# duowuyms/MANSY_ImmersiveVideoStreaming

Measured on AMD Instinct MI355X. Metric: viewport-trajectories/sec (VP train), higher is better.
Workload: dtype f32; 1 GPU; VP Transformer train step (fwd+loss+bwd+AdamW), B=4096/GPU synthetic torus-walk trajectories len 21 (hist 10 + cur 1 + pred 10), d=512, 8 heads, 2+2 layers, dropout on, fp32 MFMA, decoder recurrence as two half-batches on two streams; two_stream=True, global_batch=4096, parallelism=dp1

## Files before the change

mansy_immersivevideostreaming_amd/csrc/vp_engine.hip:

```cpp
#include <stdlib.h>
#include <algorithm>
#include <string>
#include <vector>
#include "mansy_kernels.h"
#include "../../include/mansy_hip.h"

namespace {

constexpr int MAXL = 8;

inline uint32_t site_pe_src() { return 1u; }
inline uint32_t site_enc(int l, int k) { return 100u + l * 8 + k; }
inline uint32_t site_pe_tgt(int i) { return 1000u + i; }
inline uint32_t site_dec(int l, int i, int k) { return 10000u + (l * 64 + i) * 8 + k; }

struct LinearP { const float* w = nullptr; const float* b = nullptr; float* gw = nullptr; float* gb = nullptr; };
typedef LinearP NormP;
struct EncLayerP { LinearP in_proj, out_proj, lin1, lin2; NormP n1, n2; };
struct DecLayerP { LinearP sa_in, sa_out, ca_in, ca_out, lin1, lin2; NormP n1, n2, n3; };
struct VPParams {
  LinearP emb; EncLayerP enc[MAXL]; NormP enc_norm; DecLayerP dec[MAXL]; NormP dec_norm;
  LinearP conv; NormP bn; LinearP pred;
};

struct ParamInfo { std::string name; long long numel; int ndim; long long shape[4]; };

void add_param(std::vector<ParamInfo>& v, const std::string& name, long long a, long long b = 0, long long c = 0) {
  ParamInfo p; p.name = name; p.shape[0] = a; p.shape[1] = b; p.shape[2] = c; p.shape[3] = 0;
  p.ndim = c ? 3 : (b ? 2 : 1);
  p.numel = a * (b ? b : 1) * (c ? c : 1);
  v.push_back(p);
}

std::vector<ParamInfo> param_table(const mansy_vp_config& c) {
  std::vector<ParamInfo> v;
  const long long d = c.d_model, f = c.d_ff;
  const bool hb = c.has_bias != 0;
  add_param(v, "embedding.linear.weight", d, c.in_ch);
  add_param(v, "embedding.linear.bias", d);
  auto mha = [&](const std::string& p) {
    add_param(v, p + "in_proj_weight", 3 * d, d);
    if (hb) add_param(v, p + "in_proj_bias", 3 * d);
    add_param(v, p + "out_proj.weight", d, d);
    if (hb) add_param(v, p + "out_proj.bias", d);
  };
  auto lin = [&](const std::string& p, long long o, long long i) {
    add_param(v, p + ".weight", o, i);
    if (hb) add_param(v, p + ".bias", o);
  };
  auto norm = [&](const std::string& p) {
    add_param(v, p + ".weight", d);
    if (hb) add_param(v, p + ".bias", d);
  };
  for (int l = 0; l < c.n_enc; ++l) {
    const std::string p = "transformer.encoder.layers." + std::to_string(l) + ".";
    mha(p + "self_attn.");
    lin(p + "linear1", f, d); lin(p + "linear2", d, f);
    norm(p + "norm1"); norm(p + "norm2");
  }
  norm("transformer.encoder.norm");
  for (int l = 0; l < c.n_dec; ++l) {
    const std::string p = "transformer.decoder.layers." + std::to_string(l) + ".";
    mha(p + "self_attn."); mha(p + "multihead_attn.");
    lin(p + "linear1", f, d); lin(p + "linear2", d, f);
    norm(p + "norm1"); norm(p + "norm2"); norm(p + "norm3");
  }
  norm("transformer.decoder.norm");
  add_param(v, "transformer.distill_layer.downConv.weight", d, d, 3);
  add_param(v, "transformer.distill_layer.downConv.bias", d);
  add_param(v, "transformer.distill_layer.norm.weight", d);
  add_param(v, "transformer.distill_layer.norm.bias", d);
  add_param(v, "predictor.0.weight", c.in_ch, d);
  add_param(v, "predictor.0.bias", c.in_ch);
  return v;
}

void bind_params(const mansy_vp_config& c, const float* const* params, float* const* grads, VPParams& P) {
  int k = 0;
  const bool hb = c.has_bias != 0;
  auto nextw = [&](LinearP& L, bool bias) {
    L.w = params[k]; L.gw = grads ? grads[k] : nullptr; ++k;
    if (bias) { L.b = params[k]; L.gb = grads ? grads[k] : nullptr; ++k; }
  };
  nextw(P.emb, true);
  for (int l = 0; l < c.n_enc; ++l) {
    EncLayerP& e = P.enc[l];
    nextw(e.in_proj, hb); nextw(e.out_proj, hb); nextw(e.lin1, hb); nextw(e.lin2, hb); nextw(e.n1, hb); nextw(e.n2, hb);
  }
  nextw(P.enc_norm, hb);
  for (int l = 0; l < c.n_dec; ++l) {
    DecLayerP& e = P.dec[l];
    nextw(e.sa_in, hb); nextw(e.sa_out, hb); nextw(e.ca_in, hb); nextw(e.ca_out, hb);
    nextw(e.lin1, hb); nextw(e.lin2, hb); nextw(e.n1, hb); nextw(e.n2, hb); nextw(e.n3, hb);
  }
  nextw(P.dec_norm, hb);
  nextw(P.conv, true);
  nextw(P.bn, true);
  nextw(P.pred, true);
}

struct EncBuf { float *qkv, *P, *ao, *z1, *m1, *r1, *y1, *h, *z2, *m2, *r2, *y2; };
struct DecBuf {
  float *memkv, *qkv, *P1, *ao1, *z1, *m1, *r1, *y1, *qc, *P2, *ao2, *z2, *m2, *r2, *y2, *h, *z3, *m3, *r3, *y3;
  float *dqkv, *dbr1, *dqc, *dbr2, *da, *dbr3, *dmemkv;
  float *dao2, *dS2, *Pk2;
  float *dao1, *dS1, *Pk1;
};
struct Work {
  float *src6, *cur6, *fut6, *pred_bt, *dpred_bt;
  float *x0; EncBuf enc[MAXL]; float *enc_out, *me, *re;
  float *col, *conv, *bn_mean, *bn_rstd, *mem; unsigned char* argmax; double* stats; double* dis_part;
  float *tok_all, *emb_all; DecBuf dec[MAXL]; float *dec_out, *md, *rd;
  float *t_enc, *t_dec;
  float *g_a, *g_b, *g_c, *g_wide, *g_ff;
  float *s_a, *s_b, *s_c, *s_tok;
  float *dE_all, *dz_all, *dmem;
  float *lnp_dec, *lnp_enc;
  double* loss_acc;
  unsigned short *wpl, *wpl_t;
  long long wpl_stride;
  const float* fbase; unsigned short* img;
};
struct BufInfo { std::string name; size_t off; size_t bytes; };

struct Layout {
  std::vector<BufInfo> bufs;
  size_t total = 0;
  char* base = nullptr;
  void* add(const std::string& name, size_t bytes) {
    const size_t off = (total + 255) & ~size_t(255);
    total = off + bytes;
    bufs.push_back({name, off, bytes});
    return base ? (void*)(base + off) : nullptr;
  }
  float* f(const std::string& name, size_t n) { return (float*)add(name, n * sizeof(float)); }
};

void build_layout(const mansy_vp_config& c, Layout& L, Work& W) {
  const size_t B = c.B, S = c.S, T = c.T, d = c.d_model, f = c.d_ff, H = c.n_head, C6 = c.in_ch;
  const size_t M = (S - 1) / 2 + 1, N = B * S, TB = T * B;
  W.src6 = L.f("src6", N * C6); W.cur6 = L.f("cur6", B * C6); W.fut6 = L.f("fut6", TB * C6);
  W.pred_bt = L.f("pred_bt", TB * C6); W.dpred_bt = L.f("dpred_bt", TB * C6);
  W.x0 = L.f("enc.x0", N * d);
  for (int l = 0; l < c.n_enc; ++l) {
    const std::string p = "enc" + std::to_string(l) + ".";
    EncBuf& e = W.enc[l];
    e.qkv = L.f(p + "qkv", N * 3 * d); e.P = L.f(p + "P", B * H * S * S); e.ao = L.f(p + "ao", N * d);
    e.z1 = L.f(p + "z1", N * d); e.m1 = L.f(p + "m1", N); e.r1 = L.f(p + "r1", N); e.y1 = L.f(p + "y1", N * d);
    e.h = L.f(p + "h", N * f);
    e.z2 = L.f(p + "z2", N * d); e.m2 = L.f(p + "m2", N); e.r2 = L.f(p + "r2", N); e.y2 = L.f(p + "y2", N * d);
  }
  W.enc_out = L.f("enc.out", N * d); W.me = L.f("enc.me", N); W.re = L.f("enc.re", N);
  W.col = L.f("dis.col", N * 3 * d); W.conv = L.f("dis.conv", N * d);
  W.bn_mean = L.f("dis.bn_mean", d); W.bn_rstd = L.f("dis.bn_rstd", d);
  W.mem = L.f("mem", B * M * d);
  W.argmax = (unsigned char*)L.add("dis.argmax", B * M * d);
  W.stats = (double*)L.add("dis.stats", 6 * d * sizeof(double));
  W.dis_part = (double*)L.add("dis.part", (size_t)MANSY_DISTILL_PARTS * 2 * d * sizeof(double));
  W.tok_all = L.f("tok_all", (T + 1) * B * C6);
  W.emb_all = L.f("dec.emb", TB * d);
  for (int l = 0; l < c.n_dec; ++l) {
    const std::string p = "dec" + std::to_string(l) + ".";
    DecBuf& e = W.dec[l];
    e.memkv = L.f(p + "memkv", B * M * 2 * d);
    e.qkv = L.f(p + "qkv", TB * 3 * d); e.P1 = L.f(p + "P1", TB * H * T); e.ao1 = L.f(p + "ao1", TB * d);
    e.z1 = L.f(p + "z1", TB * d); e.m1 = L.f(p + "m1", TB); e.r1 = L.f(p + "r1", TB); e.y1 = L.f(p + "y1", TB * d);
    e.qc = L.f(p + "qc", TB * d); e.P2 = L.f(p + "P2", TB * H * M); e.ao2 = L.f(p + "ao2", TB * d);
    e.z2 = L.f(p + "z2", TB * d); e.m2 = L.f(p + "m2", TB); e.r2 = L.f(p + "r2", TB); e.y2 = L.f(p + "y2", TB * d);
    e.h = L.f(p + "h", TB * f);
    e.z3 = L.f(p + "z3", TB * d); e.m3 = L.f(p + "m3", TB); e.r3 = L.f(p + "r3", TB); e.y3 = L.f(p + "y3", TB * d);
    e.dqkv = L.f(p + "dqkv", TB * 3 * d); e.dbr1 = L.f(p + "dbr1", TB * d); e.dqc = L.f(p + "dqc", TB * d);
    e.dbr2 = L.f(p + "dbr2", TB * d); e.da = L.f(p + "da", TB * f); e.dbr3 = L.f(p + "dbr3", TB * d);
    e.dmemkv = L.f(p + "dmemkv", B * M * 2 * d);
    e.dao2 = L.f(p + "dao2", TB * d); e.dS2 = L.f(p + "dS2", TB * H * M); e.Pk2 = L.f(p + "Pk2", TB * H * M);
    e.dao1 = L.f(p + "dao1", TB * d); e.dS1 = L.f(p + "dS1", TB * H * T); e.Pk1 = L.f(p + "Pk1", TB * H * T);
  }
  W.dec_out = L.f("dec.out", TB * d); W.md = L.f("dec.md", TB); W.rd = L.f("dec.rd", TB);
  W.t_enc = L.f("tmp.t_enc", N * d); W.t_dec = L.f("tmp.t_dec", B * d);
  W.g_a = L.f("tmp.g_a", N * d); W.g_b = L.f("tmp.g_b", N * d); W.g_c = L.f("tmp.g_c", N * d);
  W.g_wide = L.f("tmp.g_wide", N * 3 * d); W.g_ff = L.f("tmp.g_ff", N * f);
  W.s_a = L.f("tmp.s_a", B * d); W.s_b = L.f("tmp.s_b", B * d); W.s_c = L.f("tmp.s_c", B * d);
  W.s_tok = L.f("tmp.s_tok", B * C6);
  W.dE_all = L.f("dec.dE", TB * d); W.dz_all = L.f("dec.dz", TB * C6); W.dmem = L.f("dmem", B * M * d);
  W.lnp_dec = L.f("lnp.dec", (size_t)2 * (3 * c.n_dec + 1) * mansy_ln_bwd_parts((int)B) * 2 * d);
  W.lnp_enc = L.f("lnp.enc", (size_t)(2 * c.n_enc + 1) * mansy_ln_bwd_parts((int)N) * 2 * d);
  W.loss_acc = (double*)L.add("loss_acc", 64);
  size_t wtot = 0;
  for (const ParamInfo& pi : param_table(c))
    if (pi.ndim >= 2 && pi.shape[0] * (pi.numel / pi.shape[0]) == pi.numel && pi.numel / pi.shape[0] >= 32 && pi.shape[0] >= 32)
      wtot += ((size_t)pi.numel + 63) / 64 * 64;
  W.wpl_stride = (long long)wtot;
  W.wpl = (unsigned short*)L.add("wplanes", wtot * 2 * sizeof(unsigned short));
  W.wpl_t = (unsigned short*)L.add("wplanes_t", wtot * 2 * sizeof(unsigned short));
  const size_t floats_above = (L.total + 3) / 4;
  W.fbase = (const float*)L.base;
  W.img = (unsigned short*)L.add("bf16_images", floats_above * sizeof(unsigned short));
}

int check_cfg(const mansy_vp_config* c) {
  MANSY_REQUIRE(c, "vp: null config");
  MANSY_REQUIRE(c->B >= 1 && c->S >= 1 && c->S <= 16 && c->T >= 1 && c->T <= 16, "vp: need B>=1, 1<=S,T<=16 (got B=%d S=%d T=%d)", c->B, c->S, c->T);
  MANSY_REQUIRE(c->n_head >= 1 && c->d_model % c->n_head == 0 && c->d_model / c->n_head <= 64, "vp: d_model/n_head must be an integer <= 64");
  MANSY_REQUIRE(c->d_model % 4 == 0 && c->d_ff % 4 == 0, "vp: d_model and d_ff must be multiples of 4");
  MANSY_REQUIRE(c->n_enc >= 1 && c->n_enc <= MAXL && c->n_dec >= 1 && c->n_dec <= MAXL, "vp: 1..%d layers supported", MAXL);
  MANSY_REQUIRE(c->in_ch >= 1 && c->in_ch <= 8 && c->in_ch % 3 == 0, "vp: in_ch must be 3*in_channel <= 8");
  MANSY_REQUIRE(c->max_len >= c->S && c->max_len >= c->T, "vp: positional table too short");
  MANSY_REQUIRE(c->p_pe >= 0.f && c->p_pe < 1.f && c->p_drop >= 0.f && c->p_drop < 1.f, "vp: dropout p outside [0,1)");
  MANSY_REQUIRE(c->precision == 0 || c->precision == 1 || c->precision == 3 || c->precision == 6, "vp: precision must be MANSY_PREC_F32 (0), _BF16 (1), _BF16X3 (3) or _BF16X6 (6), got %d", c->precision);
  return MANSY_OK;
}

#define RC(expr) do { int _rc = (expr); if (_rc) return _rc; } while (0)

struct Eng {
  const mansy_vp_config& c;
  VPParams P;
  Work W;
  hipStream_t st;
  bool train;
  uint32_t seed;
  int B, S, T, d, f, H, dh, M, N, TB, C6;
  float drop_scale;

  Eng(const mansy_vp_config& cfg, hipStream_t s, bool tr, uint32_t sd) : c(cfg), st(s), train(tr), seed(sd) {
    wtab.n = 0;
    prec = c.precision;
    B = c.B; S = c.S; T = c.T; d = c.d_model; f = c.d_ff; H = c.n_head; dh = d / H; M = (S - 1) / 2 + 1;
    N = B * S; TB = T * B; C6 = c.in_ch;
    drop_scale = (train && c.p_drop > 0.f) ? 1.f / (1.f - c.p_drop) : 1.f;
  }
  MansyWPlaneTab wtab; int prec = 0;
  bool s16 = false;
  unsigned short* im(const float* p) const { return s16 ? W.img + (p - W.fbase) : nullptr; }
// ... 108 lines not shown
  }
  AttnShape self_shape(int i, int nb = -1) const {
    AttnShape s; s.nb = nb < 0 ? B : nb; s.H = H; s.Lq = 1; s.Lk = i + 1; s.dh = dh;
    s.q_bs = 3 * d; s.q_rs = 0; s.k_bs = s.v_bs = 3 * d; s.k_rs = s.v_rs = (long long)B * 3 * d;
    s.o_bs = d; s.o_rs = 0; s.scale = 1.f / sqrtf((float)dh);
    return s;
  }
  AttnShape cross_shape(int nb = -1) const {
    AttnShape s; s.nb = nb < 0 ? B : nb; s.H = H; s.Lq = 1; s.Lk = M; s.dh = dh;
    s.q_bs = d; s.q_rs = 0; s.k_bs = s.v_bs = (long long)M * 2 * d; s.k_rs = s.v_rs = 2 * d;
    s.o_bs = d; s.o_rs = 0; s.scale = 1.f / sqrtf((float)dh);
    return s;
  }

  int forward(const float* src, const float* cur, const float* pe, float* bn_rm, float* bn_rv, long long* bn_nbt, float* pred_bt) {
    RC(prepare_planes());
    RC(mansy_launch_embed_fwd(src, C6, P.emb.w, P.emb.b, pe, W.x0, N, d, S, -1, dr(site_pe_src(), c.p_pe), st, im(W.x0)));
    const float* x = W.x0;
    for (int l = 0; l < c.n_enc; ++l) {
      const EncLayerP& p = P.enc[l]; EncBuf& e = W.enc[l];
      RC(lin_fwd(x, N, d, p.in_proj.w, p.in_proj.b, 3 * d, e.qkv, 0, mansy_no_drop()));
      RC(mansy_launch_attn_fwd(e.qkv, e.qkv + d, e.qkv + 2 * d, e.ao, e.P, enc_shape(), dr(site_enc(l, 0), c.p_drop), st, attn_im()));
      RC(lin_fwd(e.ao, N, d, p.out_proj.w, p.out_proj.b, d, e.z1, 0, dr(site_enc(l, 1), c.p_drop), x));
      RC(ln_of(e.z1, p.n1, e.y1, e.m1, e.r1, N));
      RC(lin_fwd(e.y1, N, d, p.lin1.w, p.lin1.b, f, e.h, 1, dr(site_enc(l, 2), c.p_drop), nullptr, 2));
      RC(lin_fwd(e.h, N, f, p.lin2.w, p.lin2.b, d, e.z2, 0, dr(site_enc(l, 3), c.p_drop), e.y1));
      RC(ln_of(e.z2, p.n2, e.y2, e.m2, e.r2, N));
      x = e.y2;
    }
    RC(ln_fwd(x, nullptr, P.enc_norm, nullptr, W.enc_out, W.me, W.re, N));
    RC(mansy_launch_im2col3(W.enc_out, W.col, B, S, d, st, im(W.col)));
    RC(lin_fwd(W.col, N, 3 * d, P.conv.w, P.conv.b, d, W.conv, 0, mansy_no_drop()));
    DistillShape ds = {B, S, M, d, c.bn_sync_world > 1 ? c.bn_sync_world : 1, c.bn_sync_fn, c.bn_sync_user};
    RC(mansy_launch_distill_fwd(W.conv, P.bn.w, P.bn.b, bn_rm, bn_rv, bn_nbt, W.bn_mean, W.bn_rstd, W.mem, W.argmax, W.stats, ds,
                                train ? 1 : 0, c.bn_eps, c.bn_momentum, st, W.dis_part, im(W.mem)));
    for (int l = 0; l < c.n_dec; ++l) {
      const DecLayerP& p = P.dec[l];
      RC(lin_fwd(W.mem, B * M, d, p.ca_in.w + (size_t)d * d, p.ca_in.b ? p.ca_in.b + d : nullptr, 2 * d, W.dec[l].memkv, 0, mansy_no_drop(), nullptr, 1));
    }
    MANSY_HIP_CHECK(hipMemcpyAsync(W.tok_all, cur, sizeof(float) * B * C6, hipMemcpyDeviceToDevice, st));
    const bool fuse_tail = mansy_dec_tail_ok(d, C6) != 0;
    const bool split = split_ok();
    const int h0 = split ? B / 2 : B;
    if (split) RC(fork());
    for (int i = 0; i < T; ++i) {
      RC(dec_fwd_step(i, 0, h0, pe, pred_bt, fuse_tail));
      if (split) { hipStream_t keep = st; st = st2; int rc = dec_fwd_step(i, h0, B - h0, pe, pred_bt, fuse_tail); st = keep; RC(rc); }
    }
    if (split) RC(join());
    return MANSY_OK;
  }

  hipStream_t st2 = nullptr;
  bool split_ok() const { return B % 2 == 0 && ((c.two_stream == 1 && B >= 2048) || (c.two_stream == 2 && B >= 256)); }
  int fork() {
    static thread_local hipStream_t s2 = nullptr; static thread_local hipEvent_t ev_f = nullptr;
    if (!s2) { MANSY_HIP_CHECK(hipStreamCreateWithFlags(&s2, hipStreamNonBlocking)); MANSY_HIP_CHECK(hipEventCreateWithFlags(&ev_f, hipEventDisableTiming)); }
    st2 = s2;
    MANSY_HIP_CHECK(hipEventRecord(ev_f, st));
    MANSY_HIP_CHECK(hipStreamWaitEvent(st2, ev_f, 0));
    return MANSY_OK;
  }
  int join() {
    static thread_local hipEvent_t ev_j = nullptr;
    if (!ev_j) MANSY_HIP_CHECK(hipEventCreateWithFlags(&ev_j, hipEventDisableTiming));
    MANSY_HIP_CHECK(hipEventRecord(ev_j, st2));
    MANSY_HIP_CHECK(hipStreamWaitEvent(st, ev_j, 0));
    return MANSY_OK;
  }

  int dec_fwd_step(int i, int b0, int nb, const float* pe, float* pred_bt, bool fuse_tail) {
    const size_t o = (size_t)i * B + b0;
    const float* tok = W.tok_all + o * C6;
    float* emb = W.emb_all + o * d;
    float* t_dec = W.t_dec + (size_t)b0 * d;
    if (i == 0 || !fuse_tail) RC(mansy_launch_embed_fwd(tok, C6, P.emb.w, P.emb.b, pe, emb, nb, d, 1, i, dr(site_pe_tgt(i), c.p_pe, (size_t)b0 * d), st, im(emb)));
    const float* xi = emb;
    for (int l = 0; l < c.n_dec; ++l) {
      const DecLayerP& p = P.dec[l]; DecBuf& e = W.dec[l];
      float* qkv_i = e.qkv + o * 3 * d;
      const float* kv0 = e.qkv + (size_t)b0 * 3 * d;
      const float* mkv = e.memkv + (size_t)b0 * M * 2 * d;
      RC(lin_fwd(xi, nb, d, p.sa_in.w, p.sa_in.b, 3 * d, qkv_i, 0, mansy_no_drop(), nullptr, 1));
      RC(mansy_launch_attn_fwd(qkv_i, kv0 + d, kv0 + 2 * d, e.ao1 + o * d, e.P1 + o * H * T, self_shape(i, nb),
                               dr(site_dec(l, i, 0), c.p_drop, (size_t)b0 * H * (i + 1)), st, attn_im(true)));
      RC(lin_fwd(e.ao1 + o * d, nb, d, p.sa_out.w, p.sa_out.b, d, e.z1 + o * d, 0, dr(site_dec(l, i, 1), c.p_drop, (size_t)b0 * d), xi));
      RC(ln_of(e.z1 + o * d, p.n1, e.y1 + o * d, e.m1 + o, e.r1 + o, nb));
      RC(lin_fwd(e.y1 + o * d, nb, d, p.ca_in.w, p.ca_in.b, d, e.qc + o * d, 0, mansy_no_drop()));
      RC(mansy_launch_attn_fwd(e.qc + o * d, mkv, mkv + d, e.ao2 + o * d, e.P2 + o * H * M, cross_shape(nb),
                               dr(site_dec(l, i, 2), c.p_drop, (size_t)b0 * H * M), st, attn_im(true)));
      RC(lin_fwd(e.ao2 + o * d, nb, d, p.ca_out.w, p.ca_out.b, d, e.z2 + o * d, 0, dr(site_dec(l, i, 3), c.p_drop, (size_t)b0 * d), e.y1 + o * d));
      RC(ln_of(e.z2 + o * d, p.n2, e.y2 + o * d, e.m2 + o, e.r2 + o, nb));
      RC(lin_fwd(e.y2 + o * d, nb, d, p.lin1.w, p.lin1.b, f, e.h + o * f, 1, dr(site_dec(l, i, 4), c.p_drop, (size_t)b0 * f), nullptr, 2));
      if (fuse_tail && l == c.n_dec - 1) {
        RC(lin_fwd(e.h + o * f, nb, f, p.lin2.w, p.lin2.b, d, t_dec, 0, dr(site_dec(l, i, 5), c.p_drop, (size_t)b0 * d)));
        break;
      }
      RC(lin_fwd(e.h + o * f, nb, f, p.lin2.w, p.lin2.b, d, e.z3 + o * d, 0, dr(site_dec(l, i, 5), c.p_drop, (size_t)b0 * d), e.y2 + o * d));
      RC(ln_of(e.z3 + o * d, p.n3, e.y3 + o * d, e.m3 + o, e.r3 + o, nb));
      xi = e.y3 + o * d;
    }
    if (fuse_tail) {
      const DecLayerP& p = P.dec[c.n_dec - 1]; DecBuf& e = W.dec[c.n_dec - 1];
      MansyDecTailFwd tp;
      tp.a = e.y2 + o * d; tp.b = t_dec; tp.n3_w = p.n3.w; tp.n3_b = p.n3.b; tp.z3 = e.z3 + o * d; tp.y3 = e.y3 + o * d;
      tp.m3 = e.m3 + o; tp.r3 = e.r3 + o;
      tp.dn_w = P.dec_norm.w; tp.dn_b = P.dec_norm.b; tp.dec_out = W.dec_out + o * d; tp.md = W.md + o; tp.rd = W.rd + o;
      tp.pw = P.pred.w; tp.pb = P.pred.b; tp.tok_next = W.tok_all + ((size_t)(i + 1) * B + b0) * C6;
      tp.pred_bt = pred_bt ? pred_bt + ((size_t)b0 * T + i) * C6 : nullptr; tp.pred_stride = (long long)T * C6;
      const bool more = i + 1 < T;
      tp.ew = P.emb.w; tp.eb = P.emb.b; tp.pe_row = pe + (size_t)(i + 1) * d; tp.emb_next = more ? W.emb_all + ((size_t)(i + 1) * B + b0) * d : nullptr;
      tp.edrop = dr(site_pe_tgt(i + 1), c.p_pe, (size_t)b0 * d);
      tp.rows = nb; tp.C = d; tp.C6 = C6; tp.eps = c.ln_eps;
// ... 76 lines not shown
                                          dr(site_dec(l, i, 0), c.p_drop, (size_t)b0 * H * (i + 1)), st, attn_im(true)));
      } else {
        RC(lin_dx(e.dbr1 + o * d, nb, d, p.sa_out.w, d, gt, nullptr, nullptr, 1.f));
        RC(mansy_launch_attn_bwd(qkv_at(e, o), kv0 + d, kv0 + 2 * d, e.P1 + o * H * T, gt, dqkv_i, dkv0 + d, dkv0 + 2 * d,
                                 self_shape(i, nb), dr(site_dec(l, i, 0), c.p_drop, (size_t)b0 * H * (i + 1)), 1, st));
      }
      RC(lin_dx(dqkv_i, nb, 3 * d, p.sa_in.w, d, gx, gz, nullptr, 1.f));
    }
    if (!fuse_head) return mansy_launch_embed_bwd(gx, P.emb.w, W.dE_all + o * d, s_tok, C6, nb, d, dr(site_pe_tgt(i), c.p_pe, bd), st);
    if (i == 0) return mansy_launch_embed_bwd(gx, P.emb.w, W.dE_all + o * d, nullptr, C6, nb, d, dr(site_pe_tgt(0), c.p_pe, bd), st);
    return MANSY_OK;
  }
  const float* qkv_at(const DecBuf& e, size_t o) const { return e.qkv + o * 3 * d; }

  int backward(const float* src, const float* dpred_bt) {
    if (wtab.n == 0) RC(prepare_planes());
    const float ms = drop_scale;
    const bool defer_cross = mansy_attn_deferred_kv_ok(cross_shape(), T) != 0;
    const bool pull_self = mansy_attn_deferred_kv_ok(self_shape(T - 1), T) != 0;
    for (int l = 0; l < c.n_dec; ++l) {
      if (!pull_self) MANSY_HIP_CHECK(hipMemsetAsync(W.dec[l].dqkv, 0, sizeof(float) * (size_t)TB * 3 * d, st));
      if (!defer_cross) MANSY_HIP_CHECK(hipMemsetAsync(W.dec[l].dmemkv, 0, sizeof(float) * (size_t)B * M * 2 * d, st));
    }
    const bool ln_parts = mansy_ln_bwd_partial_ok(d);
    const size_t lnp_set = (size_t)mansy_ln_bwd_parts(B) * 2 * d;
    const int n_ln = 3 * c.n_dec + 1;
    const bool split = split_ok();
    const int h0 = split ? B / 2 : B;
    if (ln_parts) MANSY_HIP_CHECK(hipMemsetAsync(W.lnp_dec, 0, sizeof(float) * (size_t)(split ? 2 : 1) * n_ln * lnp_set, st));
    const bool fuse_head = ln_parts && mansy_dec_tail_ok(d, C6) != 0;
    if (split) RC(fork());
    for (int i = T - 1; i >= 0; --i) {
      RC(dec_bwd_step(i, 0, h0, 0, dpred_bt, defer_cross, pull_self, ln_parts, fuse_head));
      if (split) {
        hipStream_t keep = st; st = st2;
        const int rc = dec_bwd_step(i, h0, B - h0, 1, dpred_bt, defer_cross, pull_self, ln_parts, fuse_head);
        st = keep; RC(rc);
      }
    }
    if (split) RC(join());
    if (ln_parts) {
      for (int half = 0; half < (split ? 2 : 1); ++half) {
        const int np = mansy_ln_bwd_parts(half ? B - h0 : h0);
        float* base = W.lnp_dec + (size_t)half * n_ln * lnp_set;
        for (int l = 0; l < c.n_dec; ++l) {
          ln_pending[ln_n_pending++] = MansyLnReduce{base + (size_t)(3 * l + 0) * lnp_set, np, P.dec[l].n1.gw, P.dec[l].n1.gb};
          ln_pending[ln_n_pending++] = MansyLnReduce{base + (size_t)(3 * l + 1) * lnp_set, np, P.dec[l].n2.gw, P.dec[l].n2.gb};
          ln_pending[ln_n_pending++] = MansyLnReduce{base + (size_t)(3 * l + 2) * lnp_set, np, P.dec[l].n3.gw, P.dec[l].n3.gb};
        }
        ln_pending[ln_n_pending++] = MansyLnReduce{base + (size_t)(3 * c.n_dec) * lnp_set, np, P.dec_norm.gw, P.dec_norm.gb};
      }
      RC(flush_ln());
    }
    const bool side_dw = split && c.bn_sync_world <= 1;
    if (side_dw) RC(fork());
    {
      hipStream_t keep = st;
      if (side_dw) st = st2;
      int rc = mansy_launch_outer_reduce(W.dz_all, C6, W.dec_out, TB, d, P.pred.gw, 0, nullptr, P.pred.gb, st);
      if (!rc) rc = mansy_launch_outer_reduce(W.tok_all, C6, W.dE_all, TB, d, P.emb.gw, 1, P.emb.gb, nullptr, st);
      for (int l = 0; l < c.n_dec && !rc; ++l) {
        const DecLayerP& p = P.dec[l]; DecBuf& e = W.dec[l];
        const float* x_all = l == 0 ? W.emb_all : W.dec[l - 1].y3;
        rc = lin_dw(e.dqkv, x_all, TB, 3 * d, d, p.sa_in.gw, p.sa_in.gb);
        if (!rc) rc = lin_dw(e.dbr1, e.ao1, TB, d, d, p.sa_out.gw, p.sa_out.gb);
        if (!rc) rc = lin_dw(e.dqc, e.y1, TB, d, d, p.ca_in.gw, p.ca_in.gb);
        if (!rc) rc = lin_dw(e.dbr2, e.ao2, TB, d, d, p.ca_out.gw, p.ca_out.gb);
        if (!rc) rc = lin_dw(e.da, e.y2, TB, f, d, p.lin1.gw, p.lin1.gb);
        if (!rc) rc = lin_dw(e.dbr3, e.h, TB, d, f, p.lin2.gw, p.lin2.gb);
      }
      st = keep;
      RC(rc);
    }
    for (int l = 0; l < c.n_dec; ++l) {
      const DecLayerP& p = P.dec[l]; DecBuf& e = W.dec[l];
      if (defer_cross)
        RC(mansy_launch_attn_kvgrad(e.qc, (long long)B * d, e.dao2, (long long)B * d, e.dS2, e.Pk2, e.dmemkv, e.dmemkv + d, cross_shape(), T, 0, st, attn_im()));
      RC(lin_dw(e.dmemkv, W.mem, B * M, 2 * d, d, p.ca_in.gw + (size_t)d * d, p.ca_in.gb ? p.ca_in.gb + d : nullptr, defer_cross));
      RC(lin_dx(e.dmemkv, B * M, 2 * d, p.ca_in.w + (size_t)d * d, d, W.dmem, l == 0 ? nullptr : W.dmem, nullptr, 1.f, 0, defer_cross));
    }
    DistillShape ds = {B, S, M, d, c.bn_sync_world > 1 ? c.bn_sync_world : 1, c.bn_sync_fn, c.bn_sync_user};
    RC(mansy_launch_distill_bwd(W.conv, W.dmem, W.argmax, P.bn.w, P.bn.b, W.bn_mean, W.bn_rstd, W.g_a, W.g_b, P.bn.gw, P.bn.gb, W.stats,
                                ds, st, W.dis_part, im(W.g_b)));
    RC(lin_dw(W.g_b, W.col, N, d, 3 * d, P.conv.gw, P.conv.gb));
    RC(lin_dx(W.g_b, N, d, P.conv.w, 3 * d, W.g_wide, nullptr, nullptr, 1.f));
    RC(mansy_launch_col2im3(W.g_wide, W.g_a, B, S, d, st));
    if (c.bn_sync_world > 1) RC(mansy_bn_sync_invoke(2, c.bn_sync_fn, c.bn_sync_user));
    const float* last = W.enc[c.n_enc - 1].y2;
    RC(ln_bwd(W.g_a, last, W.me, W.re, P.enc_norm, W.g_b, nullptr, mansy_no_drop(), N, -1));
    float* gx = W.g_b; float* gz = W.g_a; float* gt = W.g_c;
    for (int l = c.n_enc - 1; l >= 0; --l) {
      const EncLayerP& p = P.enc[l]; EncBuf& e = W.enc[l];
      const float* x_in = l == 0 ? W.x0 : W.enc[l - 1].y2;
      RC(ln_bwd(gx, e.z2, e.m2, e.r2, p.n2, gz, gt, dr(site_enc(l, 3), c.p_drop), N, -(2 + 2 * l)));
      RC(lin_dw(gt, e.h, N, d, f, p.lin2.gw, p.lin2.gb));
      RC(lin_dx(gt, N, d, p.lin2.w, f, W.g_ff, nullptr, e.h, ms, 2));
      RC(lin_dw(W.g_ff, e.y1, N, f, d, p.lin1.gw, p.lin1.gb));
      RC(lin_dx(W.g_ff, N, f, p.lin1.w, d, gt, gz, nullptr, 1.f));
      RC(ln_bwd(gt, e.z1, e.m1, e.r1, p.n1, gz, gx, dr(site_enc(l, 1), c.p_drop), N, -(3 + 2 * l)));
      RC(lin_dw(gx, e.ao, N, d, d, p.out_proj.gw, p.out_proj.gb));
      RC(lin_dx(gx, N, d, p.out_proj.w, d, gt, nullptr, nullptr, 1.f));
      RC(mansy_launch_attn_bwd(e.qkv, e.qkv + d, e.qkv + 2 * d, e.P, gt, W.g_wide, W.g_wide + d, W.g_wide + 2 * d, enc_shape(),
                               dr(site_enc(l, 0), c.p_drop), 0, st, attn_im()));
      RC(lin_dw(W.g_wide, x_in, N, 3 * d, d, p.in_proj.gw, p.in_proj.gb));
      RC(lin_dx(W.g_wide, N, 3 * d, p.in_proj.w, d, gx, gz, nullptr, 1.f));
    }
    RC(mansy_launch_embed_bwd(gx, P.emb.w, gt, nullptr, C6, N, d, dr(site_pe_src(), c.p_pe), st));
    RC(mansy_launch_outer_reduce(src, C6, gt, N, d, P.emb.gw, 1, P.emb.gb, nullptr, st));
    RC(flush_ln());
    if (side_dw) RC(join());
    return MANSY_OK;
  }
};

int setup(const mansy_vp_config* cfg, void* workspace, Layout& L, Work& W) {
  RC(check_cfg(cfg));
  L.base = (char*)workspace;
  build_layout(*cfg, L, W);
  return MANSY_OK;
}

}

extern "C" {

int mansy_vp_num_params(const mansy_vp_config* cfg) {
  if (check_cfg(cfg)) return MANSY_EINVAL;
  return (int)param_table(*cfg).size();
}

int mansy_vp_param_info(const mansy_vp_config* cfg, int idx, char* name, int name_len, long long* numel, int* ndim, long long shape[4]) {
  RC(check_cfg(cfg));
  const std::vector<ParamInfo> t = param_table(*cfg);
  MANSY_REQUIRE(idx >= 0 && idx < (int)t.size(), "vp_param_info: index %d out of range", idx);
  if (name && name_len > 0) { strncpy(name, t[idx].name.c_str(), name_len - 1); name[name_len - 1] = 0; }
  if (numel) *numel = t[idx].numel;
  if (ndim) *ndim = t[idx].ndim;
  if (shape) for (int i = 0; i < 4; ++i) shape[i] = t[idx].shape[i];
  return MANSY_OK;
}

size_t mansy_vp_workspace_bytes(const mansy_vp_config* cfg) {
  Layout L; Work W;
  if (setup(cfg, nullptr, L, W)) return 0;
  return L.total + 256;
}

int mansy_vp_ws_lookup(const mansy_vp_config* cfg, const char* name, long long* offset_bytes, long long* numel) {
  Layout L; Work W;
  RC(setup(cfg, nullptr, L, W));
  for (const BufInfo& b : L.bufs)
    if (b.name == name) { if (offset_bytes) *offset_bytes = (long long)b.off; if (numel) *numel = (long long)(b.bytes / 4); return MANSY_OK; }
  mansy_set_error("vp_ws_lookup: unknown buffer '%s'", name);
  return MANSY_EINVAL;
}

int mansy_vp_forward(const mansy_vp_config* cfg, const float* const* params, const float* pe, float* bn_running_mean,
                     float* bn_running_var, long long* bn_num_batches, const float* src, const float* cur, float* pred,
                     void* workspace, int train, uint32_t seed, void* stream) {
  MANSY_REQUIRE(params && pe && bn_running_mean && bn_running_var && src && cur && pred && workspace, "vp_forward: null pointer");
  Layout L; Work W;
  RC(setup(cfg, workspace, L, W));
  Eng e(*cfg, (hipStream_t)stream, train != 0, seed);
  e.W = W;
// ... 58 lines not shown
```

mansy_immersivevideostreaming_amd/viewport_prediction/models/mtio.py:

```python
import ctypes
import random
import weakref

import numpy as np
import torch
import torch.nn as nn

from ... import _lib
from ..._lib import VPConfig, check, lib, ptr, stream_ptr

_PE_MAX_LEN = 5000
_N_HEAD = 8
_ATTN_DROPOUT = 0.1


_BN_MODELS = weakref.WeakValueDictionary()


def _bn_sync_callback(which, user):
    try:
        m = _BN_MODELS[int(user or 0)]
        cfg = m._bn_cfg
        if which == 2:
            if m._grad_ready is not None:
# ... 12 lines not shown


_BN_SYNC_CFUNC = _lib.BN_SYNC_FN(_bn_sync_callback)


class _Node(nn.Module):
    """Name-space node so parameters get the reference's dotted state_dict keys."""


def _positional_table(max_len, d_model):
    import math
    pe = torch.zeros(max_len, d_model)
    position = torch.arange(0, max_len).unsqueeze(1)
    div_term = torch.exp(torch.arange(0, d_model, 2) * -(math.log(10000.0) / d_model))
    pe[:, 0::2] = torch.sin(position * div_term)
    pe[:, 1::2] = torch.cos(position * div_term)
    return pe.unsqueeze(0)


class ViewportTransformerMTIO(nn.Module):
    def __init__(self, in_channel, fut_window, d_model, dim_feedforward, num_head=3, num_encoder_layers=2,
                 num_decoder_layers=2, batch_first=True, dropout=0.2, device='cuda', repeat_prob=0.5, seed=1,
                 bias=True):
        super().__init__()
        if not batch_first:
            raise ValueError('only batch_first=True is supported (the reference never uses anything else)')
        if num_head != 3:
            raise ValueError('the HIP MTIO kernels are built for num_head=3 (reference default)')
        self.in_channel = in_channel
        self.num_head = num_head
        self.fut_window = fut_window
        self.d_model = d_model
        self.dim_feedforward = dim_feedforward
        self.num_encoder_layers = num_encoder_layers
        self.num_decoder_layers = num_decoder_layers
        self.dropout_p = float(dropout)
        self.attn_dropout_p = _ATTN_DROPOUT
        self.device = device
        self.repeat_prob = repeat_prob
        self.seed = seed
        self.has_bias = bool(bias)
        self.precision = None
        self._ws = {}
        self._flat_p = None
        self._flat_g = None
        self.bn_sync_world = 1
        self._bn_allreduce = None
        self._grad_ready = None
        self.two_stream = None
        self._build_parameters()
        self._flatten()

    def _cfg(self, B, S, inference=False):
        two = 1 if self.two_stream is None else (2 if self.two_stream else 0)
        if self.precision is not None and self.precision not in _lib.PRECISIONS:
            raise _lib.MansyError(f'unknown precision {self.precision!r}: one of f32, bf16, bf16x3, bf16x6')
        cfg = VPConfig(B=B, S=S, T=self.fut_window, d_model=self.d_model, n_head=_N_HEAD, d_ff=self.dim_feedforward,
                       n_enc=self.num_encoder_layers, n_dec=self.num_decoder_layers, in_ch=self.in_channel * self.num_head,
                       has_bias=int(self.has_bias), p_pe=self.dropout_p, p_drop=self.attn_dropout_p, ln_eps=1e-5, bn_eps=1e-5,
                       bn_momentum=0.1, max_len=_PE_MAX_LEN, bn_sync_world=int(self.bn_sync_world), two_stream=int(two),
                       precision=_lib.resolve_precision(self.precision))
        if self.bn_sync_world > 1:
            cfg.bn_sync_fn = _BN_SYNC_CFUNC
            cfg.bn_sync_user = id(self)
        return cfg

    def set_data_parallel(self, world, allreduce=None):
        self.bn_sync_world = int(world)
        if allreduce is None:
            import torch.distributed as dist
            allreduce = dist.all_reduce
        self._bn_allreduce = allreduce
        if self.bn_sync_world > 1:
            _BN_MODELS[id(self)] = self
        else:
            _BN_MODELS.pop(id(self), None)

    def _arm_bn_sync(self, cfg):
        if self.bn_sync_world > 1:
            self._bn_cfg = cfg

    def _param_table(self):
        L = lib()
        cfg = self._cfg(1, 1)
        n = L.mansy_vp_num_params(ctypes.byref(cfg))
        if n <= 0:
            check(-1, 'mansy_vp_num_params')
        out = []
        for i in range(n):
            buf = ctypes.create_string_buffer(160)
            numel, nd, shape = ctypes.c_longlong(), ctypes.c_int(), (ctypes.c_longlong * 4)()
            check(L.mansy_vp_param_info(ctypes.byref(cfg), i, buf, 160, ctypes.byref(numel), ctypes.byref(nd), shape),
                  'mansy_vp_param_info')
            out.append((buf.value.decode(), tuple(shape[:nd.value])))
        return out

    def _set_nested(self, dotted, value, buffer=False):
        parts = dotted.split('.')
        node = self
        for p in parts[:-1]:
            if p not in node._modules:
                node.add_module(p, _Node())
            node = node._modules[p]
        if buffer:
            node.register_buffer(parts[-1], value)
        else:
            node.register_parameter(parts[-1], value)
# ... 337 lines not shown
```

Measured before the change: 185,900 trajectories/s.

## Drive backward post-decoder phase from dependency-tracked two-stream schedule with aside weight grads

New measurement: 186,000 trajectories/s, median of 2. Within noise of the previous version (+0.1%).

```diff
diff --git a/mansy_immersivevideostreaming_amd/csrc/vp_engine.hip b/mansy_immersivevideostreaming_amd/csrc/vp_engine.hip
--- a/mansy_immersivevideostreaming_amd/csrc/vp_engine.hip
+++ b/mansy_immersivevideostreaming_amd/csrc/vp_engine.hip
@@ -3,11 +3,12 @@
 #include <string>
 #include <vector>
 #include "mansy_kernels.h"
+#include "vp_sched.h"
 #include "../../include/mansy_hip.h"
 
 namespace {
 
-constexpr int MAXL = 8;
+constexpr int MAXL = vp_sched::MAXL;
 
 inline uint32_t site_pe_src() { return 1u; }
 inline uint32_t site_enc(int l, int k) { return 100u + l * 8 + k; }
@@ -113,6 +114,7 @@
   float *tok_all, *emb_all; DecBuf dec[MAXL]; float *dec_out, *md, *rd;
   float *t_enc, *t_dec;
   float *g_a, *g_b, *g_c, *g_wide, *g_ff;
+  float *g_x, *g_b2, *g_c2, *g_wide2, *g_ff2;
   float *s_a, *s_b, *s_c, *s_tok;
   float *dE_all, *dz_all, *dmem;
   float *lnp_dec, *lnp_enc;
@@ -179,6 +181,8 @@
   W.t_enc = L.f("tmp.t_enc", N * d); W.t_dec = L.f("tmp.t_dec", B * d);
   W.g_a = L.f("tmp.g_a", N * d); W.g_b = L.f("tmp.g_b", N * d); W.g_c = L.f("tmp.g_c", N * d);
   W.g_wide = L.f("tmp.g_wide", N * 3 * d); W.g_ff = L.f("tmp.g_ff", N * f);
+  W.g_x = L.f("tmp.g_x", N * d); W.g_b2 = L.f("tmp.g_b2", N * d); W.g_c2 = L.f("tmp.g_c2", N * d);
+  W.g_wide2 = L.f("tmp.g_wide2", N * 3 * d); W.g_ff2 = L.f("tmp.g_ff2", N * f);
   W.s_a = L.f("tmp.s_a", B * d); W.s_b = L.f("tmp.s_b", B * d); W.s_c = L.f("tmp.s_c", B * d);
   W.s_tok = L.f("tmp.s_tok", B * C6);
   W.dE_all = L.f("dec.dE", TB * d); W.dz_all = L.f("dec.dz", TB * C6); W.dmem = L.f("dmem", B * M * d);
@@ -393,13 +397,16 @@
   }
 
   hipStream_t st2 = nullptr;
-  bool split_ok() const { return B % 2 == 0 && ((c.two_stream == 1 && B >= 2048) || (c.two_stream == 2 && B >= 256)); }
+  bool split_ok() const { return B % 2 == 0 && ((c.two_stream == 1 && B >= 2048) || ((c.two_stream == 2 || c.two_stream == 3) && B >= 256)); }
+  struct SideRes { hipStream_t s2 = nullptr; hipEvent_t ev_f = nullptr; std::vector<hipEvent_t> pool; };
+  static SideRes& side_res() { static thread_local SideRes r; return r; }
   int fork() {
-    static thread_local hipStream_t s2 = nullptr; static thread_local hipEvent_t ev_f = nullptr;
-    if (!s2) { MANSY_HIP_CHECK(hipStreamCreateWithFlags(&s2, hipStreamNonBlocking)); MANSY_HIP_CHECK(hipEventCreateWithFlags(&ev_f, hipEventDisableTiming)); }
-    st2 = s2;
-    MANSY_HIP_CHECK(hipEventRecord(ev_f, st));
-    MANSY_HIP_CHECK(hipStreamWaitEvent(st2, ev_f, 0));
+    SideRes& r = side_res();
+    if (!r.s2) MANSY_HIP_CHECK(hipStreamCreateWithFlags(&r.s2, hipStreamNonBlocking));
+    if (!r.ev_f) MANSY_HIP_CHECK(hipEventCreateWithFlags(&r.ev_f, hipEventDisableTiming));
+    st2 = r.s2;
+    MANSY_HIP_CHECK(hipEventRecord(r.ev_f, st));
+    MANSY_HIP_CHECK(hipStreamWaitEvent(st2, r.ev_f, 0));
     return MANSY_OK;
   }
   int join() {
@@ -582,64 +589,98 @@
       }
       RC(flush_ln());
     }
-    const bool side_dw = split && c.bn_sync_world <= 1;
-    if (side_dw) RC(fork());
-    {
-      hipStream_t keep = st;
-      if (side_dw) st = st2;
-      int rc = mansy_launch_outer_reduce(W.dz_all, C6, W.dec_out, TB, d, P.pred.gw, 0, nullptr, P.pred.gb, st);
-      if (!rc) rc = mansy_launch_outer_reduce(W.tok_all, C6, W.dE_all, TB, d, P.emb.gw, 1, P.emb.gb, nullptr, st);
-      for (int l = 0; l < c.n_dec && !rc; ++l) {
+    const vp_sched::Sched sch = vp_sched::build(c.n_enc, c.n_dec, split, c.bn_sync_world > 1, defer_cross, c.two_stream == 3);
+    hipEvent_t* ev = nullptr;
+    if (sch.n_events) {
+      SideRes& r = side_res();
+      if (!r.s2) MANSY_HIP_CHECK(hipStreamCreateWithFlags(&r.s2, hipStreamNonBlocking));
+      while ((int)r.pool.size() < sch.n_events) {
+        hipEvent_t e; MANSY_HIP_CHECK(hipEventCreateWithFlags(&e, hipEventDisableTiming)); r.pool.push_back(e);
+      }
+      st2 = r.s2; ev = r.pool.data();
+    }
+    hipStream_t main_st = st;
+    for (const vp_sched::Op& o : sch.ops) {
+      hipStream_t os = o.stream ? st2 : main_st;
+      for (int e : o.waits) MANSY_HIP_CHECK(hipStreamWaitEvent(os, ev[e], 0));
+      st = os;
+      const int rc = run_post_op(o, src, defer_cross);
+      st = main_st;
+      RC(rc);
+      if (o.rec >= 0) MANSY_HIP_CHECK(hipEventRecord(ev[o.rec], os));
+    }
+    return MANSY_OK;
+  }
+
+  float* sbuf(int b) const {
+    switch (b) {
+      case vp_sched::G_A: return W.g_a; case vp_sched::G_B: return W.g_b; case vp_sched::G_C: return W.g_c;
+      case vp_sched::G_WIDE: return W.g_wide; case vp_sched::G_FF: return W.g_ff; case vp_sched::G_X: return W.g_x;
+      case vp_sched::G_B2: return W.g_b2; case vp_sched::G_C2: return W.g_c2; case vp_sched::G_WIDE2: return W.g_wide2;
+      case vp_sched::G_FF2: return W.g_ff2; case vp_sched::DMEM: return W.dmem;
+      default: break;
+    }
+    if (b >= vp_sched::DMEMKV0 && b < vp_sched::DMEMKV0 + MAXL) return W.dec[b - vp_sched::DMEMKV0].dmemkv;
+    return nullptr;
+  }
+  int run_post_op(const vp_sched::Op& o, const float* src, bool defer_cross) {
+    using namespace vp_sched;
+    const float ms = drop_scale;
+    const int l = o.layer;
+    float *in0 = sbuf(o.in0), *in1 = sbuf(o.in1), *out0 = sbuf(o.out0), *out1 = sbuf(o.out1);
+    switch (o.kind) {
+      case BEGIN: case END: return MANSY_OK;
+      case DEC_PRED_DW: return mansy_launch_outer_reduce(W.dz_all, C6, W.dec_out, TB, d, P.pred.gw, 0, nullptr, P.pred.gb, st);
+      case DEC_EMB_DW: return mansy_launch_outer_reduce(W.tok_all, C6, W.dE_all, TB, d, P.emb.gw, 1, P.emb.gb, nullptr, st);
+      case DEC_DW: {
         const DecLayerP& p = P.dec[l]; DecBuf& e = W.dec[l];
-        const float* x_all = l == 0 ? W.emb_all : W.dec[l - 1].y3;
-        rc = lin_dw(e.dqkv, x_all, TB, 3 * d, d, p.sa_in.gw, p.sa_in.gb);
-        if (!rc) rc = lin_dw(e.dbr1, e.ao1, TB, d, d, p.sa_out.gw, p.sa_out.gb);
-        if (!rc) rc = lin_dw(e.dqc, e.y1, TB, d, d, p.ca_in.gw, p.ca_in.gb);
-        if (!rc) rc = lin_dw(e.dbr2, e.ao2, TB, d, d, p.ca_out.gw, p.ca_out.gb);
-        if (!rc) rc = lin_dw(e.da, e.y2, TB, f, d, p.lin1.gw, p.lin1.gb);
-        if (!rc) rc = lin_dw(e.dbr3, e.h, TB, d, f, p.lin2.gw, p.lin2.gb);
+        switch (o.sub) {
+          case 0: return lin_dw(e.dqkv, l == 0 ? W.emb_all : W.dec[l - 1].y3, TB, 3 * d, d, p.sa_in.gw, p.sa_in.gb);
+          case 1: return lin_dw(e.dbr1, e.ao1, TB, d, d, p.sa_out.gw, p.sa_out.gb);
+          case 2: return lin_dw(e.dqc, e.y1, TB, d, d, p.ca_in.gw, p.ca_in.gb);
+          case 3: return lin_dw(e.dbr2, e.ao2, TB, d, d, p.ca_out.gw, p.ca_out.gb);
+          case 4: return lin_dw(e.da, e.y2, TB, f, d, p.lin1.gw, p.lin1.gb);
+          default: return lin_dw(e.dbr3, e.h, TB, d, f, p.lin2.gw, p.lin2.gb);
+        }
       }
-      st = keep;
-      RC(rc);
-    }
-    for (int l = 0; l < c.n_dec; ++l) {
-      const DecLayerP& p = P.dec[l]; DecBuf& e = W.dec[l];
-      if (defer_cross)
-        RC(mansy_launch_attn_kvgrad(e.qc, (long long)B * d, e.dao2, (long long)B * d, e.dS2, e.Pk2, e.dmemkv, e.dmemkv + d, cross_shape(), T, 0, st, attn_im()));
-      RC(lin_dw(e.dmemkv, W.mem, B * M, 2 * d, d, p.ca_in.gw + (size_t)d * d, p.ca_in.gb ? p.ca_in.gb + d : nullptr, defer_cross));
-      RC(lin_dx(e.dmemkv, B * M, 2 * d, p.ca_in.w + (size_t)d * d, d, W.dmem, l == 0 ? nullptr : W.dmem, nullptr, 1.f, 0, defer_cross));
-    }
-    DistillShape ds = {B, S, M, d, c.bn_sync_world > 1 ? c.bn_sync_world : 1, c.bn_sync_fn, c.bn_sync_user};
-    RC(mansy_launch_distill_bwd(W.conv, W.dmem, W.argmax, P.bn.w, P.bn.b, W.bn_mean, W.bn_rstd, W.g_a, W.g_b, P.bn.gw, P.bn.gb, W.stats,
-                                ds, st, W.dis_part, im(W.g_b)));
-    RC(lin_dw(W.g_b, W.col, N, d, 3 * d, P.conv.gw, P.conv.gb));
-    RC(lin_dx(W.g_b, N, d, P.conv.w, 3 * d, W.g_wide, nullptr, nullptr, 1.f));
-    RC(mansy_launch_col2im3(W.g_wide, W.g_a, B, S, d, st));
-    if (c.bn_sync_world > 1) RC(mansy_bn_sync_invoke(2, c.bn_sync_fn, c.bn_sync_user));
-    const float* last = W.enc[c.n_enc - 1].y2;
-    RC(ln_bwd(W.g_a, last, W.me, W.re, P.enc_norm, W.g_b, nullptr, mansy_no_drop(), N, -1));
-    float* gx = W.g_b; float* gz = W.g_a; float* gt = W.g_c;
-    for (int l = c.n_enc - 1; l >= 0; --l) {
-      const EncLayerP& p = P.enc[l]; EncBuf& e = W.enc[l];
-      const float* x_in = l == 0 ? W.x0 : W.enc[l - 1].y2;
-      RC(ln_bwd(gx, e.z2, e.m2, e.r2, p.n2, gz, gt, dr(site_enc(l, 3), c.p_drop), N, -(2 + 2 * l)));
-      RC(lin_dw(gt, e.h, N, d, f, p.lin2.gw, p.lin2.gb));
-      RC(lin_dx(gt, N, d, p.lin2.w, f, W.g_ff, nullptr, e.h, ms, 2));
-      RC(lin_dw(W.g_ff, e.y1, N, f, d, p.lin1.gw, p.lin1.gb));
-      RC(lin_dx(W.g_ff, N, f, p.lin1.w, d, gt, gz, nullptr, 1.f));
-      RC(ln_bwd(gt, e.z1, e.m1, e.r1, p.n1, gz, gx, dr(site_enc(l, 1), c.p_drop), N, -(3 + 2 * l)));
-      RC(lin_dw(gx, e.ao, N, d, d, p.out_proj.gw, p.out_proj.gb));
-      RC(lin_dx(gx, N, d, p.out_proj.w, d, gt, nullptr, nullptr, 1.f));
-      RC(mansy_launch_attn_bwd(e.qkv, e.qkv + d, e.qkv + 2 * d, e.P, gt, W.g_wide, W.g_wide + d, W.g_wide + 2 * d, enc_shape(),
-                               dr(site_enc(l, 0), c.p_drop), 0, st, attn_im()));
-      RC(lin_dw(W.g_wide, x_in, N, 3 * d, d, p.in_proj.gw, p.in_proj.gb));
-      RC(lin_dx(W.g_wide, N, 3 * d, p.in_proj.w, d, gx, gz, nullptr, 1.f));
-    }
-    RC(mansy_launch_embed_bwd(gx, P.emb.w, gt, nullptr, C6, N, d, dr(site_pe_src(), c.p_pe), st));
-    RC(mansy_launch_outer_reduce(src, C6, gt, N, d, P.emb.gw, 1, P.emb.gb, nullptr, st));
-    RC(flush_ln());
-    if (side_dw) RC(join());
-    return MANSY_OK;
+      case KVGRAD: { DecBuf& e = W.dec[l];
+        return mansy_launch_attn_kvgrad(e.qc, (long long)B * d, e.dao2, (long long)B * d, e.dS2, e.Pk2, out0, out0 + d, cross_shape(), T, 0, st, attn_im()); }
+      case MEM_DW: { const DecLayerP& p = P.dec[l];
+        return lin_dw(in0, W.mem, B * M, 2 * d, d, p.ca_in.gw + (size_t)d * d, p.ca_in.gb ? p.ca_in.gb + d : nullptr, defer_cross); }
+      case MEM_DX: return lin_dx(in0, B * M, 2 * d, P.dec[l].ca_in.w + (size_t)d * d, d, out0, in1, nullptr, 1.f, 0, defer_cross);
+      case DISTILL_BWD: {
+        DistillShape ds = {B, S, M, d, c.bn_sync_world > 1 ? c.bn_sync_world : 1, c.bn_sync_fn, c.bn_sync_user};
+        return mansy_launch_distill_bwd(W.conv, in0, W.argmax, P.bn.w, P.bn.b, W.bn_mean, W.bn_rstd, out0, out1, P.bn.gw, P.bn.gb, W.stats,
+                                        ds, st, W.dis_part, im(out1));
+      }
+      case CONV_DW: return lin_dw(in0, W.col, N, d, 3 * d, P.conv.gw, P.conv.gb);
+      case CONV_DX: return lin_dx(in0, N, d, P.conv.w, 3 * d, out0, nullptr, nullptr, 1.f);
+      case COL2IM: return mansy_launch_col2im3(in0, out0, B, S, d, st);
+      case DP_HOOK: return mansy_bn_sync_invoke(2, c.bn_sync_fn, c.bn_sync_user);
+      case ENC_NORM_BWD: return ln_bwd(in0, W.enc[c.n_enc - 1].y2, W.me, W.re, P.enc_norm, out0, nullptr, mansy_no_drop(), N, -1);
+      case EMBED_BWD: return mansy_launch_embed_bwd(in0, P.emb.w, out0, nullptr, C6, N, d, dr(site_pe_src(), c.p_pe), st);
+      case ENC_EMB_DW: return mansy_launch_outer_reduce(src, C6, in0, N, d, P.emb.gw, 1, P.emb.gb, nullptr, st);
+      case FLUSH_LN: return flush_ln();
+      default: break;
+    }
+    const EncLayerP& p = P.enc[l]; EncBuf& e = W.enc[l];
+    switch (o.kind) {
+      case LN2_BWD: return ln_bwd(in0, e.z2, e.m2, e.r2, p.n2, out0, out1, dr(site_enc(l, 3), c.p_drop), N, -(2 + 2 * l));
+      case LIN2_DW: return lin_dw(in0, e.h, N, d, f, p.lin2.gw, p.lin2.gb);
+      case LIN2_DX: return lin_dx(in0, N, d, p.lin2.w, f, out0, nullptr, e.h, ms, 2);
+      case LIN1_DW: return lin_dw(in0, e.y1, N, f, d, p.lin1.gw, p.lin1.gb);
+      case LIN1_DX: return lin_dx(in0, N, f, p.lin1.w, d, out0, in1, nullptr, 1.f);
+      case LN1_BWD: return ln_bwd(in0, e.z1, e.m1, e.r1, p.n1, out0, out1, dr(site_enc(l, 1), c.p_drop), N, -(3 + 2 * l));
+      case OUT_DW: return lin_dw(in0, e.ao, N, d, d, p.out_proj.gw, p.out_proj.gb);
+      case OUT_DX: return lin_dx(in0, N, d, p.out_proj.w, d, out0, nullptr, nullptr, 1.f);
+      case ATTN_BWD: return mansy_launch_attn_bwd(e.qkv, e.qkv + d, e.qkv + 2 * d, e.P, in0, out0, out0 + d, out0 + 2 * d, enc_shape(),
+                                                  dr(site_enc(l, 0), c.p_drop), 0, st, attn_im());
+      case IN_DW: return lin_dw(in0, l == 0 ? W.x0 : W.enc[l - 1].y2, N, 3 * d, d, p.in_proj.gw, p.in_proj.gb);
+      case IN_DX: return lin_dx(in0, N, 3 * d, p.in_proj.w, d, out0, in1, nullptr, 1.f);
+      default: break;
+    }
+    mansy_set_error("vp: unknown op %d in the backward schedule", o.kind);
+    return MANSY_EINVAL;
   }
 };
 
diff --git a/mansy_immersivevideostreaming_amd/csrc/vp_sched.h b/mansy_immersivevideostreaming_amd/csrc/vp_sched.h
--- /dev/null
+++ b/mansy_immersivevideostreaming_amd/csrc/vp_sched.h
@@ -0,0 +1,144 @@
+#pragma once
+#include <vector>
+
+namespace vp_sched {
+
+constexpr int MAXL = 8;
+
+enum Kind {
+  BEGIN,
+  DEC_PRED_DW, DEC_EMB_DW, DEC_DW,
+  KVGRAD, MEM_DW, MEM_DX,
+  DISTILL_BWD, CONV_DW, CONV_DX, COL2IM,
+  DP_HOOK,
+  ENC_NORM_BWD,
+  LN2_BWD, LIN2_DW, LIN2_DX, LIN1_DW, LIN1_DX, LN1_BWD, OUT_DW, OUT_DX, ATTN_BWD, IN_DW, IN_DX,
+  EMBED_BWD, ENC_EMB_DW, FLUSH_LN,
+  END,
+  N_KINDS
+};
+
+enum Buf {
+  FWD,
+  G_A, G_B, G_C, G_WIDE, G_FF,
+  G_X, G_B2, G_C2, G_WIDE2, G_FF2,
+  DMEM, LNP,
+  GR_PRED, GR_EMB, GR_CONV, GR_BN, GR_LN,
+  DMEMKV0,
+  GR_DEC0 = DMEMKV0 + MAXL,
+  GR_MEMKV0 = GR_DEC0 + 6 * MAXL,
+  GR_ENC0 = GR_MEMKV0 + MAXL,
+  N_BUFS = GR_ENC0 + 4 * MAXL
+};
+
+enum Mode { R = 1, W = 2, A = 3 };
+struct Access { int buf; int mode; };
+inline bool conflicts(int m1, int m2) { return !(m1 == R && m2 == R) && !(m1 == A && m2 == A); }
+
+struct Op {
+  int kind = 0, layer = 0, sub = 0;
+  int stream = 0;
+  int in0 = -1, in1 = -1, out0 = -1, out1 = -1;
+  int rec = -1;
+  std::vector<int> waits;
+  std::vector<Access> acc;
+};
+
+struct Sched { std::vector<Op> ops; int n_events = 0; };
+
+inline bool ops_conflict(const Op& a, const Op& b) {
+  for (const Access& x : a.acc)
+    for (const Access& y : b.acc)
+      if (x.buf == y.buf && conflicts(x.mode, y.mode)) return true;
+  return false;
+}
+
+class Builder {
+ public:
+  Sched s;
+  Op& op(int kind, int stream, int layer = 0, int sub = 0) {
+    cur = Op(); cur.kind = kind; cur.stream = stream; cur.layer = layer; cur.sub = sub;
+    return cur;
+  }
+  Builder& in(int b, int b1 = -1) { cur.in0 = b; cur.in1 = b1; acc(b, R); if (b1 >= 0) acc(b1, R); return *this; }
+  Builder& out(int b, int b1 = -1) { cur.out0 = b; cur.out1 = b1; acc(b, W); if (b1 >= 0) acc(b1, W); return *this; }
+  Builder& acc(int b, int mode) { cur.acc.push_back({b, mode}); return *this; }
+  void push() {
+    const int me = (int)s.ops.size();
+    for (int q = me - 1; q > synced[cur.stream]; --q) {
+      Op& o = s.ops[q];
+      if (o.stream == cur.stream || !ops_conflict(o, cur)) continue;
+      if (o.rec < 0) o.rec = s.n_events++;
+      cur.waits.push_back(o.rec);
+      synced[cur.stream] = q;
+      break;
+    }
+    s.ops.push_back(cur);
+  }
+ private:
+  Op cur;
+  int synced[2] = {-1, -1};
+};
+
+inline Sched build(int n_enc, int n_dec, bool two_stream, bool dp, bool kvgrad, bool leaves_aside) {
+  const bool side = two_stream && !dp;
+  const bool aside = side && leaves_aside;
+  const int leaf = side ? 1 : 0, leaf2 = aside ? 1 : 0;
+  Builder b;
+  b.op(BEGIN, 0); b.acc(FWD, W).acc(DMEM, W).acc(LNP, W);
+  for (int i = GR_PRED; i < N_BUFS; ++i) b.acc(i, W);
+  b.push();
+  b.op(DEC_PRED_DW, leaf); b.acc(FWD, R).acc(GR_PRED, A); b.push();
+  b.op(DEC_EMB_DW, leaf); b.acc(FWD, R).acc(GR_EMB, A); b.push();
+  for (int l = 0; l < n_dec; ++l)
+    for (int k = 0; k < 6; ++k) { b.op(DEC_DW, leaf, l, k); b.acc(FWD, R).acc(GR_DEC0 + 6 * l + k, W); b.push(); }
+  auto dw = [&](int kind, int l, int operand, int grad) { b.op(kind, leaf2, l); b.in(operand).acc(FWD, R).acc(grad, W); b.push(); };
+  for (int l = 0; l < n_dec; ++l) {
+    if (kvgrad) { b.op(KVGRAD, 0, l); b.out(DMEMKV0 + l).acc(FWD, R); b.push(); }
+    if (!aside) dw(MEM_DW, l, DMEMKV0 + l, GR_MEMKV0 + l);
+    b.op(MEM_DX, 0, l); b.in(DMEMKV0 + l, l ? DMEM : -1).out(DMEM).acc(FWD, R); b.push();
+    if (aside) dw(MEM_DW, l, DMEMKV0 + l, GR_MEMKV0 + l);
+  }
+  const int dconv = aside ? G_B2 : G_B;
+  b.op(DISTILL_BWD, 0); b.in(DMEM).out(G_A, dconv).acc(FWD, R).acc(GR_BN, W); b.push();
+  if (!aside) dw(CONV_DW, 0, dconv, GR_CONV);
+  b.op(CONV_DX, 0); b.in(dconv).out(G_WIDE).acc(FWD, R); b.push();
+  if (aside) dw(CONV_DW, 0, dconv, GR_CONV);
+  b.op(COL2IM, 0); b.in(G_WIDE).out(G_A); b.push();
+  if (dp) {
+    b.op(DP_HOOK, 0); b.acc(GR_PRED, R).acc(GR_CONV, R).acc(GR_BN, R);
+    for (int l = 0; l < n_dec; ++l) { b.acc(GR_MEMKV0 + l, R); for (int k = 0; k < 6; ++k) b.acc(GR_DEC0 + 6 * l + k, R); }
+    b.push();
+  }
+  const int gz = G_A, gx = aside ? G_X : G_B, t = aside ? G_X : G_C;
+  b.op(ENC_NORM_BWD, 0); b.in(G_A).out(gx).acc(FWD, R).acc(LNP, W); b.push();
+  for (int l = n_enc - 1, j = 0; l >= 0; --l, ++j) {
+    const bool second = aside && (j & 1);
+    const int dz2 = second ? G_C2 : G_C, dz1 = second ? G_B2 : G_B, ff = second ? G_FF2 : G_FF, wide = second ? G_WIDE2 : G_WIDE;
+    b.op(LN2_BWD, 0, l); b.in(gx).out(gz, dz2).acc(FWD, R).acc(LNP, W); b.push();
+    if (!aside) dw(LIN2_DW, l, dz2, GR_ENC0 + 4 * l + 3);
+    b.op(LIN2_DX, 0, l); b.in(dz2).out(ff).acc(FWD, R); b.push();
+    if (aside) dw(LIN2_DW, l, dz2, GR_ENC0 + 4 * l + 3);
+    if (!aside) dw(LIN1_DW, l, ff, GR_ENC0 + 4 * l + 2);
+    b.op(LIN1_DX, 0, l); b.in(ff, gz).out(t).acc(FWD, R); b.push();
+    if (aside) dw(LIN1_DW, l, ff, GR_ENC0 + 4 * l + 2);
+    b.op(LN1_BWD, 0, l); b.in(t).out(gz, dz1).acc(FWD, R).acc(LNP, W); b.push();
+    if (!aside) dw(OUT_DW, l, dz1, GR_ENC0 + 4 * l + 1);
+    b.op(OUT_DX, 0, l); b.in(dz1).out(t).acc(FWD, R); b.push();
+    if (aside) dw(OUT_DW, l, dz1, GR_ENC0 + 4 * l + 1);
+    b.op(ATTN_BWD, 0, l); b.in(t).out(wide).acc(FWD, R); b.push();
+    if (!aside) dw(IN_DW, l, wide, GR_ENC0 + 4 * l + 0);
+    b.op(IN_DX, 0, l); b.in(wide, gz).out(gx).acc(FWD, R); b.push();
+    if (aside) dw(IN_DW, l, wide, GR_ENC0 + 4 * l + 0);
+  }
+  const int demb = aside ? G_A : G_C;
+  b.op(EMBED_BWD, 0); b.in(gx).out(demb).acc(FWD, R); b.push();
+  b.op(ENC_EMB_DW, 0); b.in(demb).acc(FWD, R).acc(GR_EMB, A); b.push();
+  b.op(FLUSH_LN, 0); b.acc(LNP, R).acc(GR_LN, W); b.push();
+  b.op(END, 0);
+  for (int i = GR_PRED; i < N_BUFS; ++i) b.acc(i, R);
+  b.push();
+  return b.s;
+}
+
+}
diff --git a/mansy_immersivevideostreaming_amd/viewport_prediction/models/mtio.py b/mansy_immersivevideostreaming_amd/viewport_prediction/models/mtio.py
--- a/mansy_immersivevideostreaming_amd/viewport_prediction/models/mtio.py
+++ b/mansy_immersivevideostreaming_amd/viewport_prediction/models/mtio.py
@@ -88,7 +88,7 @@
         self._flatten()
 
     def _cfg(self, B, S, inference=False):
-        two = 1 if self.two_stream is None else (2 if self.two_stream else 0)
+        two = 1 if self.two_stream is None else (3 if self.two_stream == 'leaves' else (2 if self.two_stream else 0))
         if self.precision is not None and self.precision not in _lib.PRECISIONS:
             raise _lib.MansyError(f'unknown precision {self.precision!r}: one of f32, bf16, bf16x3, bf16x6')
         cfg = VPConfig(B=B, S=S, T=self.fut_window, d_model=self.d_model, n_head=_N_HEAD, d_ff=self.dim_feedforward,
```
